# YuePanEdward/MULLS

Hardware: NVIDIA H100
Metric: scan-pair registrations/sec (120k-pt 64-beam) (higher is better)
Workload: dtype f32 geometry / f64 accumulation

## Files before the change

### mulls_b200/csrc/kernels_iterate.cuh

```cuda
#pragma once
#include <cooperative_groups.h>

#include "device_math.cuh"
#include "device_types.cuh"
#include "kernels_ingest.cuh"

namespace mulls {

__device__ __forceinline__ bool chunk_in_run(const DeviceArrays &A) { return blockIdx.x < (unsigned)A.ctl->n_it_chunks; }
__device__ __forceinline__ int loop_buf(const DeviceArrays &A, int buf) { return buf >= 0 ? buf : (A.ctl->it & 1); }
__device__ __forceinline__ mulls_icp_trace *trace_of(const DeviceArrays &A, uint32_t pair) {
    return (A.trace && A.ctl->trace_on) ? &A.trace[pair] : nullptr;
}

template <class Body>
__device__ __forceinline__ void for_each_live_chunk(const DeviceArrays &A, int parity, int which, Body body) {
    __shared__ uint32_t s_fetch;
    LoopCtl &ctl = *A.ctl;
    const uint32_t n = ctl.n_live[parity];
    const uint32_t *list = A.live_chunks + (size_t)parity * A.live_stride;
    for (;;) {
        __syncthreads();
        if (threadIdx.x == 0) s_fetch = atomicAdd(&ctl.work[which], 1u);
        __syncthreads();
// ... 332 lines not shown
        s_pass[threadIdx.x >> 5] = __popc(pb);
    }
    __syncthreads();
    if (threadIdx.x == 0) {
        unsigned k = 0, p = 0;
        for (int w = 0; w < kIterBlock / 32; ++w) {
            k += s_kept[w];
            p += s_pass[w];
        }
        A.blk_kept[chunk] = k;
        if (p) atomicAdd(&ps.n_corr[c], p);
    }
}
constexpr int kResolveBlocksPerSm = 16;
__global__ void __launch_bounds__(kIterBlock, kResolveBlocksPerSm) k_resolve(DeviceArrays A, int buf) {
    buf = loop_buf(A, buf);
    for_each_live_chunk(A, buf, 1, [&](uint32_t chunk) { resolve_body(A, buf, chunk); });
}

template <class Sink>
__device__ __forceinline__ void terms_pt2pl(const float4 p, const float pi, const float4 q, const float4 qn,
                                            float weight, int iter_num, bool dist_w, bool resid_w, bool inten_w,
                                            float window, Sink t, float &w_out) {
    const float px = p.x, py = p.y, pz = p.z, qx = q.x, qy = q.y, qz = q.z;
    const float ntx = qn.x, nty = qn.y, ntz = qn.z;
    float w = weight;
    const float a = ntz * py - nty * pz;
    const float b = ntx * pz - ntz * px;
    const float c = nty * px - ntx * py;
    const float d = ntx * qx + nty * qy + ntz * qz - ntx * px - nty * py - ntz * pz;
    const float dist = sqrtf(qx * qx + qy * qy + qz * qz);
    if (dist_w) w = w * weight_by_dist_adaptive(dist, iter_num);
    if (resid_w) w = w * weight_by_residual(fabsf(d), window);
    if (inten_w) w = w * weight_by_intensity((float)((double)pi + 0.0001), (float)((double)q.w + 0.0001));
    w_out = w;
    t[0] = w * ntx * ntx;
    t[1] = w * ntx * nty;
    t[2] = w * ntx * ntz;
    t[3] = w * a * ntx;
    t[4] = w * b * ntx;
    t[5] = w * c * ntx;
    t[6] = w * nty * nty;
    t[7] = w * nty * ntz;
    t[8] = w * a * nty;
    t[9] = w * b * nty;
    t[10] = w * c * nty;
    t[11] = w * ntz * ntz;
    t[12] = w * a * ntz;
    t[13] = w * b * ntz;
    t[14] = w * c * ntz;
    t[15] = w * a * a;
    t[16] = w * a * b;
    t[17] = w * a * c;
    t[18] = w * b * b;
    t[19] = w * b * c;
    t[20] = w * c * c;
    t[21] = w * d * ntx;
    t[22] = w * d * nty;
    t[23] = w * d * ntz;
    t[24] = w * d * a;
    t[25] = w * d * b;
    t[26] = w * d * c;
}

__device__ __forceinline__ int diag_index(int j) {
    const int d[6] = {0, 6, 11, 15, 18, 20};
    return d[j];
}

template <class Sink>
__device__ __forceinline__ void terms_pt2li(const float4 p, const float pi, const float4 q, const float4 qv,
                                            float weight, int iter_num, bool dist_w, bool resid_w, bool inten_w,
                                            float window, Sink t, float &w_out) {
    const float px = p.x, py = p.y, pz = p.z, qx = q.x, qy = q.y, qz = q.z;
    const float vx = qv.x, vy = qv.y, vz = qv.z;
    const float dx = px - qx, dy = py - qy, dz = pz - qz;
    double Am[3][6], bv[3];
    Am[0][0] = 0;
    Am[0][1] = (double)(-vz);
    Am[0][2] = (double)vy;
    Am[0][3] = (double)(vy * py + vz * pz);
    Am[0][4] = (double)(-vy * px);
    Am[0][5] = (double)(-vz * px);
    Am[1][0] = (double)vz;
    Am[1][1] = 0;
    Am[1][2] = (double)(-vx);
    Am[1][3] = (double)(-vx * py);
    Am[1][4] = (double)(vz * pz + vx * px);
    Am[1][5] = (double)(-vz * py);
    Am[2][0] = (double)(-vy);
    Am[2][1] = (double)vx;
    Am[2][2] = 0;
    Am[2][3] = (double)(-vx * pz);
    Am[2][4] = (double)(-vy * pz);
    Am[2][5] = (double)(vx * px + vy * py);
    bv[0] = (double)(-vy * dz + vz * dy);
    bv[1] = (double)(-vz * dx + vx * dz);
    bv[2] = (double)(-vx * dy + vy * dx);
    const float ex = (float)fabs(bv[0]), ey = (float)fabs(bv[1]), ez = (float)fabs(bv[2]);
    const float ed = sqrtf(ex * ex + ey * ey + ez * ez);
    float wx = weight;
    const float dist = sqrtf(qx * qx + qy * qy + qz * qz);
    if (dist_w) wx = wx * weight_by_dist_adaptive(dist, iter_num);
    if (inten_w) wx = wx * weight_by_intensity((float)((double)pi + 0.0001), (float)((double)q.w + 0.0001));
    if (resid_w) wx = wx * weight_by_residual(ed, window);
    w_out = wx;
    const double sw = (double)sqrtf(wx);
#pragma unroll
    for (int r = 0; r < 3; ++r) {
#pragma unroll
        for (int cc = 0; cc < 6; ++cc) Am[r][cc] = sw * Am[r][cc];
        bv[r] = sw * bv[r];
    }
#pragma unroll
    for (int k = 0; k < 21; ++k) t[k] = 0.0;
    const int dg[6] = {0, 6, 11, 15, 18, 20};
#pragma unroll
    for (int j = 0; j < 6; ++j) {
        t[dg[j]] = Am[0][j] * Am[0][j] + (Am[1][j] * Am[1][j] + Am[2][j] * Am[2][j]);
        t[21 + j] = Am[0][j] * bv[0] + (Am[1][j] * bv[1] + Am[2][j] * bv[2]);
    }
}

template <class Sink>
__device__ __forceinline__ void terms_pt2pt(const float4 p, const float pi, const float4 q, float weight,
                                            int iter_num, bool dist_w, bool resid_w, bool inten_w, float window,
                                            Sink t) {
    const float px = p.x, py = p.y, pz = p.z, qx = q.x, qy = q.y, qz = q.z;
    const float dx = px - qx, dy = py - qy, dz = pz - qz;
    float wx = weight;
    const float dist = sqrtf(qx * qx + qy * qy + qz * qz);
    if (dist_w) wx = wx * weight_by_dist_adaptive(dist, iter_num);
    if (resid_w) wx = wx * weight_by_residual(sqrtf(dx * dx + dy * dy + dz * dz), window);
    if (inten_w) wx = wx * weight_by_intensity((float)((double)pi + 0.0001), (float)((double)q.w + 0.0001));
    const float wy = wx, wz = wx;
#pragma unroll
    for (int k = 0; k < 27; ++k) t[k] = 0.0;
    t[0] = wx;
    t[4] = wx * pz;
    t[5] = (-wx * py);
    t[6] = wy;
    t[8] = (-wy * pz);
    t[10] = wy * px;
    t[11] = wz;
    t[12] = wz * py;
    t[13] = (-wz * px);
    t[15] = wy * pz * pz + wz * py * py;
    t[16] = (-wz * px * py);
    t[17] = (-wy * px * pz);
    t[18] = wx * pz * pz + wz * px * px;
    t[19] = (-wx * py * pz);
    t[20] = wx * py * py + wy * px * px;
    t[21] = (-wx * dx);
    t[22] = (-wy * dy);
    t[23] = (-wz * dz);
    t[24] = wy * pz * dy - wz * py * dz;
    t[25] = wz * px * dz - wx * pz * dx;
    t[26] = wx * py * dx - wy * px * dy;
}

__device__ __forceinline__ float balanced_ground_weight(const PairConst &pc, const uint32_t *n_corr) {
    if (!pc.w_balance) return 1.0f;
    const int m1 = (int)(n_corr[MULLS_GROUND] + n_corr[MULLS_ROOF]);
    const int m2 = (int)n_corr[MULLS_FACADE], m3 = (int)n_corr[MULLS_PILLAR], m4 = (int)n_corr[MULLS_BEAM];
    const float num = pc.z_xy_ratio * (float)(m2 + 2 * m3 - m4);
    const double v = (double)num / (0.0001 + 2.0 * (double)m1);
    return (float)((0.01 > v) ? 0.01 : v);
}

__device__ __forceinline__ bool too_few(const PairConst &pc, const PairState &ps, const uint32_t *n_corr, float &ratio) {
    int total = 0;
    for (int c = 0; c < kNumClasses; ++c) total += (int)n_corr[c];
    const int nec = (int)(n_corr[MULLS_PILLAR] + n_corr[MULLS_BEAM] + n_corr[MULLS_FACADE]);
    ratio = (float)(1.0 * (double)nec / (double)ps.source_feature_points_count);
    return total < 40 || nec < 20 || ratio < pc.min_ratio;
}

__device__ __forceinline__ void pair_left_running(DeviceArrays &A) {
    const int left = atomicSub(A.running, 1) - 1;
    *A.h_running = left;
    __threadfence_system();
}

__device__ __noinline__ void solve_and_advance(DeviceArrays &A, uint32_t pair, const double *S, double *sm ,
                                  int buf_written) {
    const PairConst &pc = A.pc[pair];
    PairState &ps = A.ps[pair];
    const int i = ps.iter;
    ps.iters_entered = i + 1;
    for (int c = 0; c < kNumClasses; ++c) ps.n_corr_last[c] = ps.n_corr[c];
    {
        uint64_t pts = 0;
        for (int c = 0; c < kNumClasses; ++c)
            if (pc.used[c]) pts += (uint64_t)ps.n_tgt[c];
        ps.alg_bytes += 28ull * pts;
    }
    mulls_icp_trace *tr = trace_of(A, pair);
    if (tr && i < MULLS_MAX_TRACE_ITERS) {
        tr->n_iter = i + 1;
        for (int c = 0; c < kNumClasses; ++c) tr->n_corr[i][c] = ps.n_corr[c];
        for (int k = 0; k < 36; ++k) tr->atpa[i][k] = 0.0;
        for (int k = 0; k < 6; ++k) tr->atpb[i][k] = tr->x[i][k] = 0.0;
    }
    float ratio;
    const bool few = too_few(pc, ps, ps.n_corr, ratio);
    ps.confidence = ratio;
    if (few) {
        ps.code = -2;
        ps.status = kDone;
        pair_left_running(A);
        return;
    }
    {
        const double t = 1.0 * (double)ps.thre / (double)pc.thre_rate;
        ps.thre = (t > (double)pc.thre_min) ? (float)t : pc.thre_min;
    }
    double *ATPA = sm;
    double *ATPb = sm + 36;
    double *inv = sm + 42;
    double *lu = sm + 78;
    double *Tmp = sm + 114;
    double low[21];
    for (int k = 0; k < 21; ++k) low[k] = 0.0;
    for (int k = 0; k < 6; ++k) ATPb[k] = 0.0;
    const int order[6] = {MULLS_GROUND, MULLS_FACADE, MULLS_ROOF, MULLS_PILLAR, MULLS_BEAM, MULLS_VERTEX};
    for (int o = 0; o < 6; ++o) {
        const double *s = S + order[o] * kTerms;
        for (int k = 0; k < 21; ++k) low[k] += s[k];
        for (int k = 0; k < 6; ++k) ATPb[k] += s[21 + k];
    }
    {
        int k = 0;
        for (int col = 0; col < 6; ++col)
            for (int row = col; row < 6; ++row, ++k) {
                ATPA[6 * row + col] = low[k];
                ATPA[6 * col + row] = low[k];
            }
    }
    inverse6(ATPA, inv, lu);
    double x[6];
    for (int r = 0; r < 6; ++r) {
        double s = inv[6 * r] * ATPb[0];
        for (int cc = 1; cc < 6; ++cc) s = s + inv[6 * r + cc] * ATPb[cc];
        x[r] = s;
        ps.x[r] = s;
    }
    if (tr && i < MULLS_MAX_TRACE_ITERS) {
        for (int k = 0; k < 36; ++k) tr->atpa[i][k] = ATPA[k];
        for (int k = 0; k < 6; ++k) {
            tr->atpb[i][k] = ATPb[k];
            tr->x[i][k] = x[k];
        }
    }
    {
        const float sr = (float)sin(0.5 * x[3]), sp = (float)sin(0.5 * x[4]), sy = (float)sin(0.5 * x[5]);
        const float cr = (float)cos(0.5 * x[3]), cp = (float)cos(0.5 * x[4]), cy = (float)cos(0.5 * x[5]);
        double J[3][3];
        J[0][0] = 0.5 * (double)(cr * cp * cy + sr * sp * sy);
        J[0][1] = 0.5 * (double)(-sr * sp * cy - cr * cp * sy);
        J[0][2] = 0.5 * (double)(-sr * cp * sy - cr * sp * cy);
        J[1][0] = 0.5 * (double)(-sr * sp * cy + cr * cp * sy);
        J[1][1] = 0.5 * (double)(cr * cp * cy - sr * sp * sy);
        J[1][2] = 0.5 * (double)(-cr * sp * sy + sr * cp * cy);
        J[2][0] = 0.5 * (double)(-sr * cp * sy - cr * sp * cy);
        J[2][1] = 0.5 * (double)(-cr * sp * sy - sr * cp * cy);
        J[2][2] = 0.5 * (double)(cr * cp * cy + sr * sp * sy);
        double *cof = ps.cofactor;
        for (int k = 0; k < 36; ++k) cof[k] = inv[k];
        double tmp[3][3];
        for (int r = 0; r < 3; ++r)
            for (int cc = 0; cc < 3; ++cc)
                tmp[r][cc] = J[r][0] * inv[6 * 3 + 3 + cc] + J[r][1] * inv[6 * 4 + 3 + cc] + J[r][2] * inv[6 * 5 + 3 + cc];
        for (int r = 0; r < 3; ++r)
            for (int cc = 0; cc < 3; ++cc)
                cof[6 * (3 + r) + 3 + cc] = tmp[r][0] * J[cc][0] + tmp[r][1] * J[cc][1] + tmp[r][2] * J[cc][2];
        for (int r = 0; r < 3; ++r)
            for (int cc = 0; cc < 3; ++cc)
                cof[6 * r + 3 + cc] = inv[6 * r + 3] * J[cc][0] + inv[6 * r + 4] * J[cc][1] + inv[6 * r + 5] * J[cc][2];
        for (int r = 0; r < 3; ++r)
            for (int cc = 0; cc < 3; ++cc)
                cof[6 * (3 + r) + cc] = J[r][0] * inv[6 * 3 + cc] + J[r][1] * inv[6 * 4 + cc] + J[r][2] * inv[6 * 5 + cc];
    }
    double *Tt = ps.T_inc;
    construct_trans_a(x, Tt);
    const double ts_norm = sqrt(Tt[3] * Tt[3] + Tt[7] * Tt[7] + Tt[11] * Tt[11]);
    const double rs_angle = fabs(rotation_angle(Tt));
    if (ts_norm > (double)pc.max_t || rs_angle > (double)pc.max_r) {
        ps.code = -1;
        ps.status = kDone;
        pair_left_running(A);
        return;
    }
    mat4_mul(Tt, ps.T_total, Tmp);
    for (int k = 0; k < 16; ++k) ps.T_total[k] = Tmp[k];
    if (i == pc.max_iter - 1 || (i > 2 && ts_norm < (double)pc.conv_t && rs_angle < (double)pc.conv_r)) {
        ps.status = kNeedPosterior;
        ps.final_buf = buf_written;
        pair_left_running(A);
        return;
    }
    ps.iter = i + 1;
}

template <class Emit>
__device__ __forceinline__ void accumulate_source(DeviceArrays &A, const PairConst &pc, const PairState &ps, int c,
                                                  int buf, int it, uint32_t gi, uint32_t gd, uint32_t fl, bool few,
                                                  const uint32_t *n_corr, Emit emit) {
    const bool kept = (fl & 1) != 0, pass = (fl & 2) != 0;
    float4 p = make_float4(0, 0, 0, 0);
    int j = -1;
    float d2 = 0.0f;
    if (kept) {
        p = advanced_pos(ps, A.src_pos[buf][gi]);
        j = A.nn_idx[gi];
        d2 = A.nn_d2[gi];
        if (j >= 0) A.claim[pc.tgt_base[c] + j] = kClaimFree;
        A.src_pos[buf ^ 1][gd] = p;
        A.src_nrm[buf ^ 1][gd] = advanced_nrm(ps, A.src_nrm[buf][gi]);
        A.src_prevj[buf ^ 1][gd] = j;
        if (it >= kKeepFromIter - 1) A.src_cert[buf ^ 1][gd] = A.src_cert[buf][gi];
    }
    float w_store = 0.0f;
    double t[27];
    if (pass && !few) {
        const float4 q = A.tgt_pos[pc.tgt_base[c] + j];
        const float4 qn = A.tgt_nrm[pc.tgt_base[c] + j];
        const bool resid_w = pc.w_residual && it > 2;
        const bool dist_w = pc.w_dist != 0, inten_w = pc.w_intensity != 0;
        if (c == MULLS_GROUND || c == MULLS_FACADE || c == MULLS_ROOF) {
            const float wc = (c == MULLS_FACADE) ? 1.0f : balanced_ground_weight(pc, n_corr);
            terms_pt2pl(p, p.w, q, qn, wc, it, dist_w, resid_w, inten_w, pc.win_pt2pl, t, w_store);
            emit(t);
        } else if (c == MULLS_PILLAR || c == MULLS_BEAM) {
            terms_pt2li(p, p.w, q, qn, 1.0f, it, dist_w, resid_w, inten_w, pc.win_pt2li, t, w_store);
            emit(t);
        } else {
            terms_pt2pt(p, p.w, q, 1.0f, it, dist_w, resid_w, inten_w, pc.win_pt2pt, t);
            w_store = d2;
            emit(t);
        }
    } else {
        constexpr double kZeros[27] = {};
        emit(kZeros);
    }
    if (kept) {
        A.corr_j[gd] = pass ? j : -1;
        A.corr_w[gd] = w_store;
    }
}

constexpr int kAccumulateBlocksPerSm = 4;
__device__ __forceinline__ void accumulate_chunk_warp(DeviceArrays &A, int buf, uint32_t chunk) {
    const ChunkDesc cd = A.it_chunks[chunk];
    const PairConst &pc = A.pc[cd.pair];
    PairState &ps = A.ps[cd.pair];
    if (ps.status != kRunning) return;
    const int c = (int)cd.seg;
    const int ns = ps.n_src[c];
    if ((int)cd.first >= ns) return;
    const int lane = threadIdx.x & 31;
    constexpr int kSlots = kIterBlock / 32;
    const uint32_t first = pc.src_base[c] + cd.first;
    uint32_t fl = 0;
#pragma unroll
    for (int s = 0; s < kSlots; ++s)
        if ((int)cd.first + 32 * s + lane < ns) fl |= (uint32_t)A.flags[first + 32 * s + lane] << (8 * s);
    uint32_t dst = 0;
#pragma unroll 4
    for (uint32_t b = pc.class_chunk_begin[c] + lane; b < chunk; b += 32) dst += A.blk_kept[b];
    for (int o = 16; o > 0; o >>= 1) dst += __shfl_xor_sync(0xffffffffu, dst, o);
    uint32_t n_corr[kNumClasses];
#pragma unroll
    for (int k = 0; k < kNumClasses; ++k) n_corr[k] = ps.n_corr[k];
    float ratio_unused;
    const bool few = too_few(pc, ps, n_corr, ratio_unused);
    const int it = ps.iter;
    double acc[27];
#pragma unroll
    for (int k = 0; k < 27; ++k) acc[k] = -0.0;
#pragma unroll 1
    for (int s = 0; s < kSlots; ++s, fl >>= 8) {
        const unsigned kb = __ballot_sync(0xffffffffu, (fl & 1) != 0);
        const uint32_t gd = pc.src_base[c] + dst + __popc(kb & ((1u << lane) - 1u));
        dst += __popc(kb);
        accumulate_source(A, pc, ps, c, buf, it, first + 32 * s + lane, gd, fl, few, n_corr, [&acc](const double *t) {
#pragma unroll
            for (int k = 0; k < 27; ++k) acc[k] += t[k];
        });
    }
    double mine = 0.0;
#pragma unroll
    for (int k = 0; k < 27; ++k) {
        double v = acc[k];
#pragma unroll
        for (int o = 16; o > 0; o >>= 1) v += __shfl_xor_sync(0xffffffffu, v, o);
        if (lane == k) mine = v;
    }
    if (lane < 27) A.partials[(size_t)chunk * kTerms + lane] = mine;
}
__global__ void __launch_bounds__(kIterBlock, kAccumulateBlocksPerSm) k_accumulate(DeviceArrays A, int buf) {
    buf = loop_buf(A, buf);
    LoopCtl &ctl = *A.ctl;
    if (blockIdx.x == 0 && threadIdx.x == 0) ctl.work[0] = 0u;
    const uint32_t n = ctl.n_live[buf];
    const uint32_t *list = A.live_chunks + (size_t)buf * A.live_stride;
    for (;;) {
        uint32_t w = 0;
        if ((threadIdx.x & 31) == 0) w = atomicAdd(&ctl.work[2], 1u);
        w = __shfl_sync(0xffffffffu, w, 0);
        if (w >= n) break;
        accumulate_chunk_warp(A, buf, list[w]);
    }
}

__device__ __forceinline__ void accumulate_chunk_block(DeviceArrays &A, int buf, uint32_t chunk) {
    const ChunkDesc cd = A.it_chunks[chunk];
    const PairConst &pc = A.pc[cd.pair];
    PairState &ps = A.ps[cd.pair];
    if (ps.status != kRunning) return;
    const int c = (int)cd.seg;
    const int ns = ps.n_src[c];
    const uint32_t local = cd.first + threadIdx.x;
    const bool valid = (int)local < ns;
    const int lane = threadIdx.x & 31, warp = threadIdx.x >> 5;
    constexpr int kWarps = kIterBlock / 32;
    __shared__ double s_terms[27 * kIterBlock];
    __shared__ uint32_t s_off[kWarps + 1];
    __shared__ uint32_t s_base;

    if ((int)cd.first >= ns) return;
    uint8_t fl = 0;
    uint32_t gi = 0;
    {
        uint32_t acc = 0;
        const uint32_t first_chunk = pc.class_chunk_begin[c];
        for (uint32_t b = first_chunk + threadIdx.x; b < chunk; b += kIterBlock) acc += A.blk_kept[b];
        for (int o = 16; o > 0; o >>= 1) acc += __shfl_xor_sync(0xffffffffu, acc, o);
        if (lane == 0) s_off[warp] = acc;
        __syncthreads();
        if (threadIdx.x == 0) {
            uint32_t tt = 0;
            for (int w = 0; w < kWarps; ++w) tt += s_off[w];
            s_base = tt;
        }
        __syncthreads();
    }
    if (valid) {
        gi = pc.src_base[c] + local;
        fl = A.flags[gi];
    }
    const unsigned kb = __ballot_sync(0xffffffffu, (fl & 1) != 0);
    if (lane == 0) s_off[warp] = __popc(kb);
    __syncthreads();
    if (threadIdx.x == 0) {
        uint32_t run = 0;
        for (int w = 0; w < kWarps; ++w) {
            const uint32_t tt = s_off[w];
            s_off[w] = run;
            run += tt;
        }
        s_off[kWarps] = run;
    }
    __syncthreads();
    const uint32_t gd = pc.src_base[c] + s_base + s_off[warp] + __popc(kb & ((1u << lane) - 1u));
    uint32_t n_corr[kNumClasses];
#pragma unroll
    for (int k = 0; k < kNumClasses; ++k) n_corr[k] = ps.n_corr[k];
    float ratio_unused;
    const bool few = too_few(pc, ps, n_corr, ratio_unused);
    accumulate_source(A, pc, ps, c, buf, ps.iter, gi, gd, fl, few, n_corr, [](const double *t) {
#pragma unroll
        for (int k = 0; k < 27; ++k) s_terms[k * kIterBlock + threadIdx.x] = t[k];
    });
    __syncthreads();
#pragma unroll 1
    for (int k = warp; k < 27; k += kWarps) {
        const double *row = s_terms + k * kIterBlock;
        double v = ((row[lane] + row[lane + 32]) + row[lane + 64]) + row[lane + 96];
#pragma unroll
        for (int o = 16; o > 0; o >>= 1) v += __shfl_xor_sync(0xffffffffu, v, o);
        if (lane == 0) A.partials[(size_t)chunk * kTerms + k] = v;
    }
}

__device__ __forceinline__ void publish_live_chunks(const DeviceArrays &A, uint32_t pair, int next_parity) {
    __shared__ uint32_t s_base;
    __syncthreads();
    const PairConst &pc = A.pc[pair];
    const PairState &ps = A.ps[pair];
    if (ps.status != kRunning) return;
    uint32_t count[kNumClasses], total = 0;
#pragma unroll
    for (int c = 0; c < kNumClasses; ++c) {
        count[c] = (uint32_t)((ps.n_src[c] + kIterBlock - 1) / kIterBlock);
        total += count[c];
    }
    if (threadIdx.x == 0) s_base = atomicAdd(&A.ctl->n_live[next_parity], total);
    __syncthreads();
    uint32_t base = s_base;
#pragma unroll
    for (int c = 0; c < kNumClasses; ++c) {
        append_live_chunks(A, next_parity, pc.class_chunk_begin[c], count[c], base);
        base += count[c];
    }
}

__device__ __forceinline__ void solve_body(DeviceArrays &A, int buf, uint32_t pair) {
    const PairConst &pc = A.pc[pair];
    PairState &ps = A.ps[pair];
    if (ps.status != kRunning) return;
    const int lane = threadIdx.x & 31, warp = threadIdx.x >> 5, n_warps = blockDim.x >> 5;
    __shared__ double s_S[kNumClasses][kTerms];
    __shared__ double s_scratch[160];
    __shared__ int s_newn[kNumClasses];
    __shared__ uint32_t s_ncorr[kNumClasses];
    for (int cc = warp; cc < kNumClasses; cc += n_warps) {
        const uint32_t b0 = pc.class_chunk_begin[cc];
        const uint32_t live = (uint32_t)((ps.n_src[cc] + kIterBlock - 1) / kIterBlock);
        const uint32_t b1 = min(pc.class_chunk_begin[cc + 1], b0 + live);
        double a0 = 0.0, a1 = 0.0, a2 = 0.0, a3 = 0.0;
        if (lane < 27) {
            uint32_t b = b0;
            for (; b + 4 <= b1; b += 4) {
                a0 += A.partials[(size_t)(b + 0) * kTerms + lane];
                a1 += A.partials[(size_t)(b + 1) * kTerms + lane];
                a2 += A.partials[(size_t)(b + 2) * kTerms + lane];
                a3 += A.partials[(size_t)(b + 3) * kTerms + lane];
            }
            for (; b < b1; ++b) a0 += A.partials[(size_t)b * kTerms + lane];
        }
        if (lane < kTerms) s_S[cc][lane] = (lane < 27) ? ((a0 + a1) + (a2 + a3)) : 0.0;
        uint32_t acc = 0;
        for (uint32_t b = b0 + lane; b < b1; b += 32) acc += A.blk_kept[b];
        for (int o = 16; o > 0; o >>= 1) acc += __shfl_xor_sync(0xffffffffu, acc, o);
        if (lane == 0) {
            s_newn[cc] = (int)acc;
            s_ncorr[cc] = ps.n_corr[cc];
        }
    }
    __syncthreads();
    if (threadIdx.x == 0) {
        uint64_t srcpts = 0;
        for (int cc = 0; cc < kNumClasses; ++cc)
            if (pc.used[cc]) srcpts += (uint64_t)ps.n_src_g[cc];
        ps.alg_bytes += 28ull * srcpts;
        if (pc.sharded) {
            for (int cc = 0; cc < kNumClasses; ++cc) {
                ps.n_src[cc] = s_newn[cc];
                for (int k = 0; k < kTerms; ++k) A.xch_f64[cc * kTerms + k] = (k < 27) ? s_S[cc][k] : 0.0;
            }
        } else {
        mulls_icp_trace *tr = trace_of(A, pair);
        for (int cc = 0; cc < kNumClasses; ++cc) {
            ps.n_src[cc] = s_newn[cc];
            ps.n_src_g[cc] = s_newn[cc];
            ps.n_corr[cc] = s_ncorr[cc];
            if (tr && ps.iter < MULLS_MAX_TRACE_ITERS) tr->n_src[ps.iter][cc] = (uint32_t)ps.n_src[cc];
        }
        solve_and_advance(A, pair, &s_S[0][0], s_scratch, buf ^ 1);
        for (int cc = 0; cc < kNumClasses; ++cc) ps.n_corr[cc] = 0;
        }
    }
    if (!pc.sharded) publish_live_chunks(A, pair, buf ^ 1);
}
constexpr int kSolveThreads = kNumClasses * 32;
__global__ void __launch_bounds__(kSolveThreads) k_solve(DeviceArrays A, int buf, unsigned long long loop_handle) {
    LoopCtl &ctl = *A.ctl;
    if (blockIdx.x >= (unsigned)ctl.n_pairs) return;
    solve_body(A, loop_buf(A, buf), blockIdx.x);
    if (loop_handle == 0ull) return;
    __syncthreads();
    if (threadIdx.x == 0) {
        __threadfence();
        if (atomicAdd(&ctl.solved, 1u) == (unsigned)ctl.n_pairs - 1u) {
            ctl.solved = 0;
            const int it = ctl.it + 1;
            ctl.it = it;
            __threadfence();
            const bool again = *(volatile int *)A.running > 0 && it < ctl.max_iter;
            cudaGraphSetConditional((cudaGraphConditionalHandle)loop_handle, again ? 1u : 0u);
        }
    }
}

__global__ void __launch_bounds__(kIterBlock, 4) k_icp_loop(DeviceArrays A) {
    namespace cg = cooperative_groups;
    cg::grid_group grid = cg::this_grid();
    LoopCtl &ctl = *A.ctl;
    __shared__ uint8_t s_need[kIterBlock];
    __shared__ float4 s_carry[kIterBlock];
    __shared__ uint32_t s_n_need;
    const int n_pairs = ctl.n_pairs, max_iter = ctl.max_iter;
    for (int it = 0; it < max_iter; ++it) {
        const int buf = it & 1;
        const uint32_t *list = A.live_chunks + (size_t)buf * A.live_stride;
        const uint32_t n_live = ctl.n_live[buf];
        if (blockIdx.x == 0 && threadIdx.x == 0) ctl.n_live[buf ^ 1] = 0u;
        const int mode = search_mode_of(it);
        for (uint32_t w = blockIdx.x; w < n_live; w += gridDim.x) {
            const uint32_t chunk = list[w];
            if (mode == 2) search_keep_chunk(A, buf, chunk, s_need, s_carry, &s_n_need);
            else if (mode == 1) search_quarter<WalkBounds>(A, buf, chunk, threadIdx.x >> 5, true);
            else search_quarter<NoBounds>(A, buf, chunk, threadIdx.x >> 5, false);
            __syncthreads();
        }
        grid.sync();
        for (uint32_t w = blockIdx.x; w < n_live; w += gridDim.x) {
            resolve_body(A, buf, list[w]);
            __syncthreads();
        }
        grid.sync();
        for (uint32_t w = blockIdx.x; w < n_live; w += gridDim.x) {
            accumulate_chunk_block(A, buf, list[w]);
            __syncthreads();
        }
        grid.sync();
        for (int pair = blockIdx.x; pair < n_pairs; pair += gridDim.x) {
            solve_body(A, buf, (uint32_t)pair);
            __syncthreads();
        }
        grid.sync();
        if (*(volatile int *)A.running <= 0) break;
    }
}

__global__ void k_shard_pack_setup(DeviceArrays A, int phase) {
    PairState &ps = A.ps[0];
    if (phase == 0) {
        for (int d = 0; d < 3; ++d) {
            A.xch_i32[d] = ps.bb_src[d];
            A.xch_i32[3 + d] = ~ps.bb_src[3 + d];
        }
    } else if (phase == 1) {
        for (int d = 0; d < 3; ++d) {
            ps.bb_src[d] = A.xch_i32[d];
            ps.bb_src[3 + d] = ~A.xch_i32[3 + d];
        }
    } else if (phase == 2) {
        for (int c = 0; c < kNumClasses; ++c) A.xch_i32[c] = ps.n_src[c];
    } else {
        const PairConst &pc = A.pc[0];
        int cnt = 0;
        for (int c = 0; c < kNumClasses; ++c) ps.n_src_g[c] = A.xch_i32[c];
        if (pc.used[MULLS_PILLAR]) cnt += ps.n_src_g[MULLS_PILLAR];
        if (pc.used[MULLS_FACADE]) cnt += ps.n_src_g[MULLS_FACADE];
        if (pc.used[MULLS_BEAM]) cnt += ps.n_src_g[MULLS_BEAM];
        ps.source_feature_points_count = cnt;
    }
}
__global__ void __launch_bounds__(kIterBlock) k_shard_counts(DeviceArrays A, int phase) {
    const PairConst &pc = A.pc[0];
    PairState &ps = A.ps[0];
    if (ps.status != kRunning) {
        if (phase == 0 && threadIdx.x < 2 * kNumClasses) A.xch_i32[threadIdx.x] = 0;
        return;
    }
    if (phase == 0) {
        __shared__ uint32_t s_w[kIterBlock / 32];
        for (int cc = 0; cc < kNumClasses; ++cc) {
            const uint32_t b0 = pc.class_chunk_begin[cc];
            const uint32_t live = (uint32_t)((ps.n_src[cc] + kIterBlock - 1) / kIterBlock);
            const uint32_t b1 = min(pc.class_chunk_begin[cc + 1], b0 + live);
            uint32_t acc = 0;
            for (uint32_t b = b0 + threadIdx.x; b < b1; b += kIterBlock) acc += A.blk_kept[b];
            for (int o = 16; o > 0; o >>= 1) acc += __shfl_xor_sync(0xffffffffu, acc, o);
            __syncthreads();
            if ((threadIdx.x & 31) == 0) s_w[threadIdx.x >> 5] = acc;
            __syncthreads();
            if (threadIdx.x == 0) {
                uint32_t tot = 0;
                for (int w = 0; w < kIterBlock / 32; ++w) tot += s_w[w];
                A.xch_i32[kNumClasses + cc] = (int)tot;
                A.xch_i32[cc] = (int)ps.n_corr[cc];
            }
        }
    } else if (threadIdx.x == 0) {
        for (int cc = 0; cc < kNumClasses; ++cc) {
            ps.n_corr[cc] = (uint32_t)A.xch_i32[cc];
            ps.n_src_g_next[cc] = A.xch_i32[kNumClasses + cc];
        }
    }
}
__global__ void k_shard_solve(DeviceArrays A, int buf, int it_flag) {
    PairState &ps = A.ps[0];
    __shared__ double s_scratch[160];
    if (threadIdx.x == 0) {
        if (ps.status != kRunning) {
            A.h_running_iter[it_flag] = *A.running;
            __threadfence_system();
        } else {
            mulls_icp_trace *tr = trace_of(A, 0);
            for (int cc = 0; cc < kNumClasses; ++cc) {
                ps.n_src_g[cc] = ps.n_src_g_next[cc];
                if (tr && ps.iter < MULLS_MAX_TRACE_ITERS) tr->n_src[ps.iter][cc] = (uint32_t)ps.n_src_g[cc];
            }
            solve_and_advance(A, 0, A.xch_f64, s_scratch, buf ^ 1);
            for (int cc = 0; cc < kNumClasses; ++cc) ps.n_corr[cc] = 0;
            A.h_running_iter[it_flag] = *A.running;
            __threadfence_system();
        }
    }
    publish_live_chunks(A, 0, buf ^ 1);
}
__global__ void k_shard_post(DeviceArrays A, int phase) {
    const PairConst &pc = A.pc[0];
    PairState &ps = A.ps[0];
    if (threadIdx.x != 0) return;
    if (phase == 0) {
        double VTPV = 0.0, nob = 0.0;
        if (ps.status == kNeedPosterior) {
            const int order[6] = {MULLS_GROUND, MULLS_FACADE, MULLS_ROOF, MULLS_PILLAR, MULLS_BEAM, MULLS_VERTEX};
            for (int o = 0; o < 6; ++o) {
                const uint32_t b0 = pc.class_chunk_begin[order[o]];
                const uint32_t live = (uint32_t)((ps.n_src[order[o]] + kIterBlock - 1) / kIterBlock);
                const uint32_t b1 = min(pc.class_chunk_begin[order[o] + 1], b0 + live);
                for (uint32_t b = b0; b < b1; ++b) {
                    VTPV += A.post_partials[2 * (size_t)b];
                    nob += A.post_partials[2 * (size_t)b + 1];
                }
            }
        }
        A.xch_f64[0] = VTPV;
        A.xch_f64[1] = nob;
    } else if (ps.status == kNeedPosterior) {
        const double sigma2 = A.xch_f64[0] / (double)((int)A.xch_f64[1] - 6);
        ps.sigma2 = sigma2;
        ps.code = (sqrt(sigma2) < pc.sigma_thre) ? 1 : -3;
        double inv[36], lu[36];
        inverse6(ps.cofactor, inv, lu);
        for (int k = 0; k < 36; ++k) ps.info[k] = (1.0 / sigma2) * inv[k];
        ps.status = kDone;
    }
}

__global__ void __launch_bounds__(kIterBlock) k_posterior(DeviceArrays A) {
    if (!chunk_in_run(A)) return;
    const ChunkDesc cd = A.it_chunks[blockIdx.x];
    const PairConst &pc = A.pc[cd.pair];
    PairState &ps = A.ps[cd.pair];
    if (ps.status != kNeedPosterior) return;
    const int c = (int)cd.seg;
    const int buf = ps.final_buf;
    if ((int)cd.first >= ps.n_src[c]) return;
    const uint32_t local = cd.first + threadIdx.x;
    const bool valid = (int)local < ps.n_src[c];
    double vtpv = 0.0;
    int nobs = 0;
    if (valid) {
        const uint32_t gi = pc.src_base[c] + local;
        const int j = A.corr_j[gi];
        if (j >= 0) {
            const float4 p = A.src_pos[buf][gi];
            const float4 q = A.tgt_pos[pc.tgt_base[c] + j];
            const float4 qn = A.tgt_nrm[pc.tgt_base[c] + j];
            const float w = A.corr_w[gi];
            const double *x = ps.x;
            const float px = p.x, py = p.y, pz = p.z, qx = q.x, qy = q.y, qz = q.z;
            if (c == MULLS_GROUND || c == MULLS_FACADE || c == MULLS_ROOF) {
                const float ntx = qn.x, nty = qn.y, ntz = qn.z;
                const float a = ntz * py - nty * pz;
                const float b = ntx * pz - ntz * px;
                const float cc = nty * px - ntx * py;
                const float d = ntx * qx + nty * qy + ntz * qz - ntx * px - nty * py - ntz * pz;
                const float residual = (float)((double)ntx * x[0] + (double)nty * x[1] + (double)ntz * x[2] +
                                               (double)a * x[3] + (double)b * x[4] + (double)cc * x[5] - (double)d);
                vtpv = (double)(w * residual * residual);
                nobs = 1;
            } else {
                const float dx = px - qx, dy = py - qy, dz = pz - qz;
                double Am[3][6], bv[3];
                if (c == MULLS_PILLAR || c == MULLS_BEAM) {
                    const float vx = qn.x, vy = qn.y, vz = qn.z;
                    Am[0][0] = 0, Am[0][1] = (double)vz, Am[0][2] = (double)(-vy), Am[0][3] = (double)(-vz * pz - vy * py),
                    Am[0][4] = (double)(vy * px), Am[0][5] = (double)(vz * px);
                    Am[1][0] = (double)(-vz), Am[1][1] = 0, Am[1][2] = (double)vx, Am[1][3] = (double)(vx * py),
                    Am[1][4] = (double)(-vx * px - vz * pz), Am[1][5] = (double)(vz * py);
// ... 138 lines not shown
```

Before: 6580.

## Batch kept-source and target loads ahead of term computation in accumulate kernels

Restructures accumulate so each warp issues all per-slot source loads, a fixed batch of kept-count prefix loads, and target point/normal gathers up front, then stages positions and targets in shared memory before the double-precision term loop. The goal is more memory-level parallelism, so that dependent global loads no longer serialize inside each slot iteration. The block variant gets the same load-first ordering. This costs extra registers for the KeptSource arrays and a sizable shared-memory staging area per block, which may lower occupancy under the 4-blocks-per-SM launch bound.

```diff
diff --git a/mulls_b200/csrc/kernels_iterate.cuh b/mulls_b200/csrc/kernels_iterate.cuh
--- a/mulls_b200/csrc/kernels_iterate.cuh
+++ b/mulls_b200/csrc/kernels_iterate.cuh
@@ -658,29 +658,52 @@
     ps.iter = i + 1;
 }
 
+struct KeptSource {
+    float4 pos, nrm;
+    float4 cert;
+    int j;
+    float d2;
+};
+__device__ __forceinline__ KeptSource load_kept(const DeviceArrays &A, int buf, int it, uint32_t gi, bool kept) {
+    KeptSource s;
+    s.pos = s.nrm = s.cert = make_float4(0, 0, 0, 0);
+    s.j = -1;
+    s.d2 = 0.0f;
+    if (kept) {
+        s.pos = A.src_pos[buf][gi];
+        s.nrm = A.src_nrm[buf][gi];
+        s.j = A.nn_idx[gi];
+        s.d2 = A.nn_d2[gi];
+        if (it >= kKeepFromIter - 1) s.cert = A.src_cert[buf][gi];
+    }
+    return s;
+}
+__device__ __forceinline__ void load_target(const DeviceArrays &A, uint32_t tb, int j, bool live, float4 &q, float4 &qn) {
+    q = qn = make_float4(0, 0, 0, 0);
+    if (live) {
+        q = A.tgt_pos[tb + j];
+        qn = A.tgt_nrm[tb + j];
+    }
+}
+__device__ __forceinline__ void move_kept(const PairState &ps, KeptSource &s) {
+    s.pos = advanced_pos(ps, s.pos);
+    s.nrm = advanced_nrm(ps, s.nrm);
+}
+__device__ __forceinline__ void store_kept(DeviceArrays &A, uint32_t tb, int buf, int it, uint32_t gd, bool pass,
+                                           const KeptSource &s) {
+    if (s.j >= 0) A.claim[tb + s.j] = kClaimFree;
+    A.src_pos[buf ^ 1][gd] = s.pos;
+    A.src_nrm[buf ^ 1][gd] = s.nrm;
+    A.src_prevj[buf ^ 1][gd] = s.j;
+    if (it >= kKeepFromIter - 1) A.src_cert[buf ^ 1][gd] = s.cert;
+    A.corr_j[gd] = pass ? s.j : -1;
+}
 template <class Emit>
-__device__ __forceinline__ void accumulate_source(DeviceArrays &A, const PairConst &pc, const PairState &ps, int c,
-                                                  int buf, int it, uint32_t gi, uint32_t gd, uint32_t fl, bool few,
-                                                  const uint32_t *n_corr, Emit emit) {
-    const bool kept = (fl & 1) != 0, pass = (fl & 2) != 0;
-    float4 p = make_float4(0, 0, 0, 0);
-    int j = -1;
-    float d2 = 0.0f;
-    if (kept) {
-        p = advanced_pos(ps, A.src_pos[buf][gi]);
-        j = A.nn_idx[gi];
-        d2 = A.nn_d2[gi];
-        if (j >= 0) A.claim[pc.tgt_base[c] + j] = kClaimFree;
-        A.src_pos[buf ^ 1][gd] = p;
-        A.src_nrm[buf ^ 1][gd] = advanced_nrm(ps, A.src_nrm[buf][gi]);
-        A.src_prevj[buf ^ 1][gd] = j;
-        if (it >= kKeepFromIter - 1) A.src_cert[buf ^ 1][gd] = A.src_cert[buf][gi];
-    }
+__device__ __forceinline__ float source_terms(const PairConst &pc, int c, int it, bool live, const float4 p, float d2,
+                                              const float4 q, const float4 qn, const uint32_t *n_corr, Emit emit) {
     float w_store = 0.0f;
     double t[27];
-    if (pass && !few) {
-        const float4 q = A.tgt_pos[pc.tgt_base[c] + j];
-        const float4 qn = A.tgt_nrm[pc.tgt_base[c] + j];
+    if (live) {
         const bool resid_w = pc.w_residual && it > 2;
         const bool dist_w = pc.w_dist != 0, inten_w = pc.w_intensity != 0;
         if (c == MULLS_GROUND || c == MULLS_FACADE || c == MULLS_ROOF) {
@@ -699,14 +722,16 @@
         constexpr double kZeros[27] = {};
         emit(kZeros);
     }
-    if (kept) {
-        A.corr_j[gd] = pass ? j : -1;
-        A.corr_w[gd] = w_store;
-    }
+    return w_store;
 }
 
 constexpr int kAccumulateBlocksPerSm = 4;
-__device__ __forceinline__ void accumulate_chunk_warp(DeviceArrays &A, int buf, uint32_t chunk) {
+constexpr int kPrefixLoads = 8;
+struct TermStage {
+    float4 p[kIterBlock], q[kIterBlock], qn[kIterBlock];
+    uint32_t gd[kIterBlock];
+};
+__device__ __forceinline__ void accumulate_chunk_warp(DeviceArrays &A, int buf, uint32_t chunk, TermStage &st) {
     const ChunkDesc cd = A.it_chunks[chunk];
     const PairConst &pc = A.pc[cd.pair];
     PairState &ps = A.ps[cd.pair];
@@ -716,33 +741,61 @@
     if ((int)cd.first >= ns) return;
     const int lane = threadIdx.x & 31;
     constexpr int kSlots = kIterBlock / 32;
-    const uint32_t first = pc.src_base[c] + cd.first;
+    const uint32_t tb = pc.tgt_base[c], first = pc.src_base[c] + cd.first;
+    const int it = ps.iter;
     uint32_t fl = 0;
 #pragma unroll
     for (int s = 0; s < kSlots; ++s)
         if ((int)cd.first + 32 * s + lane < ns) fl |= (uint32_t)A.flags[first + 32 * s + lane] << (8 * s);
+    const uint32_t b_lane = pc.class_chunk_begin[c] + lane;
+    uint32_t kept_before[kPrefixLoads];
+#pragma unroll
+    for (int k = 0; k < kPrefixLoads; ++k) kept_before[k] = (b_lane + 32 * k < chunk) ? A.blk_kept[b_lane + 32 * k] : 0u;
+    KeptSource src[kSlots];
+#pragma unroll
+    for (int s = 0; s < kSlots; ++s) src[s] = load_kept(A, buf, it, first + 32 * s + lane, ((fl >> (8 * s)) & 1) != 0);
     uint32_t dst = 0;
-#pragma unroll 4
-    for (uint32_t b = pc.class_chunk_begin[c] + lane; b < chunk; b += 32) dst += A.blk_kept[b];
+#pragma unroll
+    for (int k = 0; k < kPrefixLoads; ++k) dst += kept_before[k];
+    for (uint32_t b = b_lane + 32 * kPrefixLoads; b < chunk; b += 32) dst += A.blk_kept[b];
     for (int o = 16; o > 0; o >>= 1) dst += __shfl_xor_sync(0xffffffffu, dst, o);
     uint32_t n_corr[kNumClasses];
 #pragma unroll
     for (int k = 0; k < kNumClasses; ++k) n_corr[k] = ps.n_corr[k];
+#pragma unroll
+    for (int s = 0; s < kSlots; ++s) move_kept(ps, src[s]);
+#pragma unroll
+    for (int s = 0; s < kSlots; ++s) {
+        const bool kept = ((fl >> (8 * s)) & 1) != 0;
+        const unsigned kb = __ballot_sync(0xffffffffu, kept);
+        const uint32_t gd = pc.src_base[c] + dst + __popc(kb & ((1u << lane) - 1u));
+        dst += __popc(kb);
+        if (kept) store_kept(A, tb, buf, it, gd, ((fl >> (8 * s)) & 2) != 0, src[s]);
+        st.gd[32 * s + lane] = gd;
+    }
     float ratio_unused;
     const bool few = too_few(pc, ps, n_corr, ratio_unused);
-    const int it = ps.iter;
+#pragma unroll
+    for (int s = 0; s < kSlots; ++s) {
+        float4 q, qn;
+        load_target(A, tb, src[s].j, ((fl >> (8 * s)) & 2) && !few, q, qn);
+        qn.w = src[s].d2;
+        st.p[32 * s + lane] = src[s].pos;
+        st.q[32 * s + lane] = q;
+        st.qn[32 * s + lane] = qn;
+    }
     double acc[27];
 #pragma unroll
     for (int k = 0; k < 27; ++k) acc[k] = -0.0;
 #pragma unroll 1
     for (int s = 0; s < kSlots; ++s, fl >>= 8) {
-        const unsigned kb = __ballot_sync(0xffffffffu, (fl & 1) != 0);
-        const uint32_t gd = pc.src_base[c] + dst + __popc(kb & ((1u << lane) - 1u));
-        dst += __popc(kb);
-        accumulate_source(A, pc, ps, c, buf, it, first + 32 * s + lane, gd, fl, few, n_corr, [&acc](const double *t) {
-#pragma unroll
-            for (int k = 0; k < 27; ++k) acc[k] += t[k];
-        });
+        const float4 qn = st.qn[32 * s + lane];
+        const float w = source_terms(pc, c, it, (fl & 2) && !few, st.p[32 * s + lane], qn.w, st.q[32 * s + lane], qn,
+                                     n_corr, [&acc](const double *t) {
+#pragma unroll
+                                         for (int k = 0; k < 27; ++k) acc[k] += t[k];
+                                     });
+        if (fl & 1) A.corr_w[st.gd[32 * s + lane]] = w;
     }
     double mine = 0.0;
 #pragma unroll
@@ -755,6 +808,7 @@
     if (lane < 27) A.partials[(size_t)chunk * kTerms + lane] = mine;
 }
 __global__ void __launch_bounds__(kIterBlock, kAccumulateBlocksPerSm) k_accumulate(DeviceArrays A, int buf) {
+    __shared__ TermStage s_stage[kIterBlock / 32];
     buf = loop_buf(A, buf);
     LoopCtl &ctl = *A.ctl;
     if (blockIdx.x == 0 && threadIdx.x == 0) ctl.work[0] = 0u;
@@ -765,7 +819,7 @@
         if ((threadIdx.x & 31) == 0) w = atomicAdd(&ctl.work[2], 1u);
         w = __shfl_sync(0xffffffffu, w, 0);
         if (w >= n) break;
-        accumulate_chunk_warp(A, buf, list[w]);
+        accumulate_chunk_warp(A, buf, list[w], s_stage[threadIdx.x >> 5]);
     }
 }
 
@@ -824,10 +878,18 @@
     for (int k = 0; k < kNumClasses; ++k) n_corr[k] = ps.n_corr[k];
     float ratio_unused;
     const bool few = too_few(pc, ps, n_corr, ratio_unused);
-    accumulate_source(A, pc, ps, c, buf, ps.iter, gi, gd, fl, few, n_corr, [](const double *t) {
+    const int it = ps.iter;
+    const bool kept = (fl & 1) != 0, live = (fl & 2) && !few;
+    KeptSource src = load_kept(A, buf, it, gi, kept);
+    float4 q, qn;
+    load_target(A, pc.tgt_base[c], src.j, live, q, qn);
+    move_kept(ps, src);
+    if (kept) store_kept(A, pc.tgt_base[c], buf, it, gd, (fl & 2) != 0, src);
+    const float w = source_terms(pc, c, it, live, src.pos, src.d2, q, qn, n_corr, [](const double *t) {
 #pragma unroll
         for (int k = 0; k < 27; ++k) s_terms[k * kIterBlock + threadIdx.x] = t[k];
     });
+    if (kept) A.corr_w[gd] = w;
     __syncthreads();
 #pragma unroll 1
     for (int k = warp; k < 27; k += kWarps) {
```

Result: no change. 6686 (median of 6 runs) (+1.6%).
